# Sudo42b/vision.cpp

Measured on AMD Instinct MI355X. Metric: images/sec, Depth-Anything-V2-Small 518x518 f16, higher is better.
Workload: dtype f16; 1 GPU; Depth-Anything-V2-Small f16 (DINOv2-S ViT) 518x518 batch=32 per MI355X (BASELINE.json configs[1]); global_batch=32, weights=random-init synthetic GGUF (seed 0), parallelism=dp1 (image shards, no data-path collective), hip_graph=True

## Files before the change

### include/visp_hip_kernels.h

```cpp
#ifndef VISP_HIP_KERNELS_H
#define VISP_HIP_KERNELS_H

#include <stddef.h>
#include <stdint.h>

#ifdef __cplusplus
extern "C" {
#endif

#define VX_API __attribute__((visibility("default")))

VX_API const char* vx_last_error(void);
VX_API int vx_device_count(void);
VX_API int vx_set_device(int index);
VX_API int vx_device_info(int index, char* name, int name_cap, char* arch, int arch_cap,
                          size_t* total_mem, size_t* free_mem, int* n_cu);
VX_API int vx_malloc(void** ptr, size_t bytes);
VX_API int vx_free(void* ptr);
VX_API int vx_memset(void* ptr, int value, size_t bytes, void* stream);
VX_API int vx_memcpy_h2d(void* dst, const void* host_src, size_t bytes, void* stream);
VX_API int vx_memcpy_d2h(void* host_dst, const void* src, size_t bytes, void* stream);
VX_API int vx_memcpy_d2d(void* dst, const void* src, size_t bytes, void* stream);
VX_API int vx_malloc_host(void** ptr, size_t bytes);
VX_API int vx_free_host(void* ptr);
VX_API int vx_memcpy_h2d_async(void* dst, const void* pinned_src, size_t bytes, void* stream);
VX_API int vx_memcpy_d2h_async(void* pinned_dst, const void* src, size_t bytes, void* stream);
VX_API int vx_event_sync(void* ev);
VX_API int vx_stream_create(void** stream);
VX_API int vx_stream_destroy(void* stream);
VX_API int vx_stream_sync(void* stream);
VX_API int vx_event_create(void** ev);
VX_API int vx_event_destroy(void* ev);
VX_API int vx_event_record(void* ev, void* stream);
VX_API int vx_event_elapsed_ms(void* start, void* stop, float* ms);
VX_API int vx_stream_wait_event(void* stream, void* ev);
VX_API int vx_graph_begin_capture(void* stream);
VX_API int vx_graph_end_capture(void* stream, void** graph_exec);
VX_API int vx_graph_launch(void* graph_exec, void* stream);
VX_API int vx_graph_destroy(void* graph_exec);

enum vx_epilogue {
    VX_EPI_F16 = 0,
    VX_EPI_F16_GELU = 1,
    VX_EPI_F16_RELU = 2,
    VX_EPI_RESID_F32 = 3,
    VX_EPI_TOKENS = 4,
    VX_EPI_QKV = 5,
    VX_EPI_PIXSHUF = 6,
    VX_EPI_F16_ADD = 7,
    VX_EPI_HEAD_OUT = 8,
    VX_EPI_LRELU_AGC = 9,
    VX_EPI_SILU = 10,
};

typedef struct {
    const void* A;
    int64_t lda;
    int a_group;
    int a_group_stride;
    int a_row_off;
    int conv_kh, conv_kw, conv_stride, conv_pad;
    int conv_H, conv_W, conv_Cin, conv_OH, conv_OW;
    int a_relu;

    const void* W;
    const float* bias;
    int M, N, K;

    int epi;
    void* out;
    int64_t ldo;
    int relu;
    const float* lambda;
    const float* pos;
    int tokens_P;
    void* q; void* k; void* vt;
    int qkv_T, qkv_Tp, qkv_H;
    float q_scale;
    int ps_s, ps_Cout, ps_H, ps_W;
    const void* res1; const void* res2;
    int n_valid;
    int stages;
    float head_bias, head_scale;
    int post_gelu, win_ws, win_res;
    int win_res_h, win_shift;
    int k_splits; float* k_partial;
    void* debug_stamps;
    const float* noise;
    int noise_hw;
    int64_t conv_pix;
    int64_t ld_res1;
} vx_gemm_args;

VX_API int vx_gemm_f16(const vx_gemm_args* args, void* stream);
VX_API int vx_gemm_pick_k_splits(int M, int N, int K);

VX_API int vx_conv3x3_supported(const vx_gemm_args* args);
VX_API int vx_conv3x3_f16(const vx_gemm_args* args, void* stream);

enum { VX_DC_F16 = 0, VX_DC_RGB_F32 = 1, VX_DC_HEAD_F32 = 2 };
typedef struct {
    const void* x; int64_t x_plane; int cin; int up2;
    int B, H, W;
    const void* w; const float* bias; int cout;
    int epi, act;
    float s1; const void* res1; int64_t res1_plane;
    float s2; const void* res2; int64_t res2_plane;
    void* out; int64_t out_plane;
    int x_residual;
    int64_t x_pix, out_pix, res1_pix, res2_pix;
    int a_relu;
    const float* head_w; float head_bias, head_scale;
    void* stamps;
    int bil_hs, bil_ws;
    int res2_hs, res2_ws;
} vx_dconv_args;
VX_API int vx_dconv_bilinear_supported(int cout, int H, int W, int hs, int ws);
VX_API int vx_dconv3x3_f16(const vx_dconv_args* args, void* stream);
VX_API int vx_dconv_prepare(void);
VX_API int vx_dconv_x_residual_supported(float s1, int act, int a_relu);
VX_API int vx_dconv_set_block_cap(int n);
VX_API void vx_dconv_set_resident_mode(int mode);

typedef struct {
    const void* x; const void* w1; const float* b1; const void* w2; const float* b2;
    const void* res2; const void* wp; const float* bp;
    void* out;
    int B, H, W;
} vx_rcu_args;
VX_API int vx_rcu_supported(int H, int W);
VX_API int vx_rcu_fused_f16(const vx_rcu_args* args, void* stream);

typedef struct { int image_w, image_h, overlap_x, overlap_y, n_x, n_y, tile_w, tile_h; } vx_tile_layout;
VX_API int vx_esrgan_tiles_in(const uint8_t* img, int B, int w, int h, int format, const vx_tile_layout* t, void* out, void* stream);
VX_API int vx_esrgan_tiles_in_f32(const uint8_t* img, int B, int w, int h, int format, const vx_tile_layout* t, float* out, void* stream);
VX_API int vx_esrgan_tiles_out(const float* tiles, int B, const vx_tile_layout* t, float* out_f32, uint8_t* out_rgba, void* stream);

VX_API int vx_tv_preprocess(const uint8_t* rgb, void* out, int64_t n_pixels, void* stream);
VX_API int vx_dwconv3x3_f16(const void* x, const void* w, const float* bias, void* y, int B, int H, int W, int C, int stride, int gelu, void* stream);
VX_API int vx_mbconv_dw_pw_supported(int C, int Cout, int W);
VX_API int vx_mbconv_pack_w3(const void* w3_rows_host, void* packed_host);
VX_API int vx_mbconv_dw_pw_f16(const void* h, const void* w2, const float* b2, const void* w3, const float* b3, const void* x, void* y, int B, int H,
                               int W, int C, int Cout, void* stream);
VX_API int vx_layernorm_f16(const void* x, const float* w, const float* b, void* y, int64_t rows_out, int C, float eps, int res, int ws,
                            int out_f32, void* stream);
VX_API size_t vx_window_attention_bias_bytes(int N, int heads);
VX_API int vx_window_attention_pack_bias(const float* bias_host, int N, int heads, void* packed_host);
VX_API int vx_window_attention_f16(const void* qkv, const void* bias_packed, void* out, int n_windows, int N, int heads, void* stream);
VX_API int vx_swin_attention_pack_bias(const float* table , int ws, int heads, void* packed_host );
VX_API int vx_window_attention_masked_f16(const void* qkv, const void* bias_packed, void* out, int n_windows, int N, int heads, int nwx, int nwy,
                                          void* stream);
VX_API int vx_swin_layernorm_f16(const void* x, const float* w, const float* b, void* y, int64_t rows_out, int C, float eps, int H, int W, int ws,
                                 int shift, int out_f32, void* stream);
VX_API int vx_swin_layernorm_strided_f16(const void* x, const float* w, const float* b, void* y, int64_t rows, int C, float eps, int ldy, int out_f32,
                                         void* stream);
VX_API int vx_swin_merge_layernorm_f16(const void* x, const float* w, const float* b, void* y, int B, int H, int W, int C, float eps, void* stream);
VX_API int vx_swin_window_reverse_add_f16(const void* a, const void* x, void* y, int B, int H, int W, int C, int ws, int shift, void* stream);
VX_API int vx_window_reverse_add_f16(const void* a, const void* x, void* y, int B, int res, int ws, int C, void* stream);
VX_API int vx_bf_preprocess_half(const uint8_t* rgb, void* out8, int B, int H, int W, void* stream);
VX_API int vx_bf_patches(const uint8_t* rgb, void* out, int B, int IH, int IW, int h, int w, void* stream);
VX_API int vx_bf_resize_f16(const void* src, int lds, void* dst, int ldd, int B, int h, int w, int C, int oh, int ow, void* stream);
VX_API int vx_bf_deform_cols_f16(const void* x, const void* offmod, int ldom, void* cols, int B, int h, int w, int C, int k, void* stream);
typedef struct {
    const void* x; int B, H, W, Cin;
    const void* w; int Cout, k, pad;
    const void* offset; int ld_offset;
    const void* mask; int ld_mask; int mask_mode; float mask_scale;
    const float* scale; const float* bias; int relu;
    void* out; int ldo;
} vx_deform_conv_args;
VX_API int vx_deform_conv_f16(const vx_deform_conv_args* args, void* stream);
VX_API int vx_bf_mean_f16(const void* x, int ld, void* y, float* acc_scratch , int B, int64_t n, int C, void* stream);
VX_API int vx_bf_broadcast_f16(const void* g, int ldg, void* dst, int ldd, int B, int64_t n, int C, void* stream);
VX_API int vx_bf_mul_sigmoid_f16(void* y, int ldy, const void* a, int lda, int64_t rows, int C, void* stream);
VX_API int vx_bf_sigmoid_out_f32(const void* a, int lda, float* out, int64_t n, void* stream);
VX_API int vx_add_rows_f16(const void* a, int a_is_f32, const void* b, int64_t b_period, void* y, int64_t n, void* stream);
VX_API int vx_small_attention_f16(const void* q, const void* k, const void* v, void* out, int Nq, int Nk, int heads, int hd, void* stream);
VX_API int vx_sam_interpolate(const void* src, int src_f16, int sw, int sh, int sstride, int step, void* dst, int dw, int dh, int out_u8, void* stream);
VX_API int vx_add_gelu_f16(const void* a, const void* b, void* y, int64_t n, void* stream);

#define VX_ATTN_Q_SCALE 0.18033688011112042f
VX_API int vx_attention_f16(const void* q, const void* k, const void* v, void* out, int B, int H, int T,
                            void* stream);
VX_API int vx_attention_masked_f16(const void* q, const void* k, const void* v, const void* mask, void* out, int B, int H, int T, int head_dim,
                                   int Hm, int Bm, int mask_is_f32, void* stream);
VX_API int vx_attention_cross_parts(int Tq, int Tk);
VX_API size_t vx_attention_cross_partial_bytes(int B, int H, int Tq, int Tk, int head_dim);
VX_API int vx_attention_cross_f16(const void* q, const void* k, const void* v, void* out, void* partial, size_t partial_bytes, int B, int H, int Tq, int Tk,
                                  int head_dim, float scale, void* stream);
VX_API int vx_attention_cross_step_f16(int step, const void* q, const void* k, const void* v, void* out, void* partial, size_t partial_bytes, int B, int H, int Tq,
                                       int Tk, int head_dim, float scale, void* stream);
VX_API int vx_mul_mat_f16(const void* a, const void* b, void* out, int64_t M, int N, int K, int B, int Ba, void* stream);
VX_API int vx_sincos_f16(int mode, const void* x, void* y, int64_t n, void* stream);
VX_API int vx_fourier_features_f32(const float* coords, const float* gauss, void* out, int64_t n_points, int F, void* stream);
VX_API int vx_sam_iou_head_f32(const void* tokens, int64_t row_stride, int P, const float* w0, const float* b0, const float* w1, const float* b1, const float* w2,
                               const float* b2, int K0, int N0, int N1, int N2, float* iou, int32_t* chosen, void* stream);
VX_API int vx_sam_process_masks(const void* planes, int64_t prompt_stride, int64_t plane_stride, int step, int mask_size, int n_planes, const int32_t* chosen,
                                float* scaled, int image_size, int sw, int sh, uint8_t* out, int dw, int dh, int P, void* stream);
VX_API int vx_sam_tile_rows_f16(const void* src, int64_t n, void* dst, int B, void* stream);
VX_API int vx_sam_score_planes_f16(const void* planes, int64_t prompt_stride, int64_t plane_stride, int mask_size, int n_planes, int cw, int ch, float offset,
                                   int32_t* table, float* stability, int P, void* stream);
VX_API size_t vx_sam_rank_nms_workspace_bytes(int N);
VX_API int vx_sam_rank_nms(const int32_t* table, const float* iou, int n_planes, int iou_stride, int N, float pred_iou_thresh, float stability_thresh,
                           float nms_iou_thresh, int capacity, void* workspace, size_t workspace_bytes, int32_t* flags, int32_t* rank, int32_t* keep_idx,
                           int32_t* counts, void* stream);
VX_API int vx_sam_process_masks_indexed(const void* planes, int64_t prompt_stride, int64_t plane_stride, int step, int mask_size, int n_scored, int n_prompts,
                                        const int32_t* keep_idx, const int32_t* counts, int capacity, int group, float* scaled, int image_size, int sw, int sh,
                                        uint8_t* out, int dw, int dh, void* stream);
VX_API int vx_sam_mask_stats_u8(const uint8_t* masks, int w, int h, const int32_t* keep_idx, const int32_t* counts, int capacity, int n_scored, int n_prompts,
                                const float* iou, int iou_stride, const float* stability, int32_t* info_i32, float* info_f32, void* stream);
#define VX_REGIONS_HOLES 1
#define VX_REGIONS_ISLANDS 2
#define VX_REGIONS_BOTH 3
VX_API size_t vx_mask_regions_workspace_bytes(int w, int h, int group);
VX_API int vx_mask_remove_small_regions_u8(uint8_t* masks, int w, int h, int n, const int32_t* counts, int min_area, int mode, int32_t* changed, void* workspace,
                                           size_t workspace_bytes, int group, void* stream);
VX_API int vx_sam_clean_nms_inputs(const int32_t* info_i32, const int32_t* changed, const int32_t* counts, int N, int32_t* table, float* key, void* stream);
VX_API int vx_sam_gather_clean_masks(const uint8_t* masks, int w, int h, const int32_t* info_i32, const float* info_f32, const int32_t* changed, const int32_t* keep_idx,
                                     const int32_t* first_counts, const int32_t* second_counts, int N, uint8_t* out_masks, int32_t* out_info_i32, float* out_info_f32,
                                     int32_t* out_counts, void* stream);
VX_API void vx_attention_set_fast_limit(float limit);
VX_API void vx_attention_set_waves(int waves);
VX_API void vx_attention_set_stamps(void* stamps);

typedef struct {
    const void* att; float* x;
    const void* w_mlp; const float* vec_mlp;
    const void* w_qkv; const float* vec_qkv;
    const float* vec_tap; void* feat;
    void *q, *k, *v;
    int M, T, H;
    float q_scale, eps;
    float* cap_x1;
    void* stamps;
} vx_dino_block_args;
VX_API int vx_dino_block_supported(int embed_dim, int hidden, int head_dim);
VX_API size_t vx_dino_block_mlp_bytes(void);
VX_API size_t vx_dino_block_qkv_bytes(void);
VX_API int vx_dino_block16_pack_mlp(const void* wo, const void* w1, const void* w2, void* out);
VX_API int vx_dino_block16_pack_qkv(const void* wqkv, void* out);
VX_API int vx_dino_block16_f16(const vx_dino_block_args* args, void* stream);

typedef struct {
    const void* A; const float* a_scale;
    const void* W; const float* w_scale;
    const float* bias;
    int M, N, Kp, n_valid;
    void* out; int64_t ldo;
    int act;
    const void* res;
} vx_gemm_fp8_args;
VX_API int vx_gemm_fp8_supported(int N, int K);
VX_API int vx_gemm_fp8(const vx_gemm_fp8_args* args, void* stream);
VX_API int vx_quantize_rows_e4m3(const void* x_f16, int64_t ldx, void* q, float* scale, int M, int K, int Kp, void* stream);
VX_API int vx_quantize_rows_e4m3_host(const float* w, int N, int K, int Kp, void* q_out, float* scale_out);

VX_API int vx_layernorm_f32_f16(const float* x, const float* w, const float* b, void* y, int M, int C,
                                float eps, void* stream);

VX_API int vx_preprocess_patches(const uint8_t* rgb, void* patches, int B, int H, int W, int ps, int Kp,
                                 const float mean[3], const float inv_std[3], void* stream);
VX_API int vx_preprocess_f32(const uint8_t* rgb, float* out, int B, int H, int W, const float mean[3],
                             const float inv_std[3], void* stream);
VX_API int vx_write_cls_rows(float* x, const float* cls, const float* pos, int B, int T, int C, void* stream);

VX_API int vx_bilinear_ac_f16(const void* x, void* y, int B, int H, int W, int C, int OH, int OW, void* stream);

VX_API int vx_head_out_f32(const void* x, const float* w, float bias, float max_depth, float* depth,
                           int64_t n_pixels, int C, void* stream);

VX_API size_t vx_headconv_frag_bytes(void);
VX_API int vx_headconv_set_block_cap(int n);
VX_API int vx_headconv_pack(const void* w_rows, int Kp, void* out_frag);
VX_API int vx_headconv_supported(int cin, int cout, int H, int W, int hs, int ws);
VX_API void vx_headconv_set_stamps(void* stamps);
// ... 85 lines not shown
```

### vision.cpp_amd/csrc/kernels_dconv.hip

```cpp
#include "vx_common.h"

#include <cmath>
#include <cstdlib>
#include <type_traits>

namespace {

constexpr int TRASH_BLOCKS = 1024;
__device__ __attribute__((aligned(16))) unsigned char g_dconv_trash[TRASH_BLOCKS * 8 * 1024];

constexpr int DCONV_TAB_MAX = 1280;
constexpr int CK = 32;
constexpr int PIXB = CK * 2;
constexpr int NW = 8;

struct tile_grid {
    int ncols, nrows, n_main, n_strip, strip_x0;
    __host__ __device__ tile_grid(int H, int W) {
        const int q = W / 32, rem = W % 32;
        const bool strip = rem > 0 && rem <= 16;
        ncols = q + ((rem > 16) ? 1 : 0);
        nrows = (H + 15) / 16;
        n_main = ncols * nrows;
        n_strip = strip ? (H + 31) / 32 : 0;
// ... 556 lines not shown
#pragma unroll
                for (int mi = 0; mi < MT; ++mi) {
                    const int oy = cur.y0 + out_row(cur.tws, mi), ox = cur.x0 + out_col(cur.tws);
                    if (oy < H && ox < W) {
                        float* o = reinterpret_cast<float*>(p.out) + (((long)cur.b * H + oy) * W + ox) * 3;
                        o[0] = acc[mi][0][0];
                        o[1] = acc[mi][0][1];
                        o[2] = acc[mi][0][2];
                    }
                }
            }
            wait_vmcnt<0>();
            prev_halo = false;
        } else {
            asm volatile("" ::: "memory");
            __builtin_amdgcn_s_barrier();
            asm volatile("" ::: "memory");
            unsigned char* st;
            if constexpr (COUT == 32) st = smem + done * HALO_BYTES + wave * 64 * PITCH;
            else st = (wave < 4 ? smem + done * HALO_BYTES : smem + W_BASE + WSt * W_BYTES) + (wave & 3) * 64 * PITCH;
            auto stage_tile = [&](auto act_c) {
                constexpr int ACT = decltype(act_c)::value;
#pragma unroll
                for (int mi = 0; mi < MT; ++mi) {
                    const int ml = mi * 32 + r;
#pragma unroll
                    for (int ni = 0; ni < NI; ++ni)
#pragma unroll
                        for (int g = 0; g < 4; ++g) {
                            const int nl = ni * 32 + 8 * g + 4 * h;
                            float4 bias = {0.f, 0.f, 0.f, 0.f};
                            if constexpr (COUT != 32) bias = *reinterpret_cast<const float4*>(s_bias + nl);
                            float v[4] = {acc[mi][ni][4 * g + 0] + bias.x, acc[mi][ni][4 * g + 1] + bias.y,
                                          acc[mi][ni][4 * g + 2] + bias.z, acc[mi][ni][4 * g + 3] + bias.w};
#pragma unroll
                            for (int j = 0; j < 4; ++j) {
                                if constexpr (ACT == 2) v[j] = relu1(v[j]);
                                else if constexpr (ACT == 1) v[j] = fmaxf(v[j], 0.2f * v[j]);
                            }
                            if (xres) {
#pragma unroll
                                for (int j = 0; j < 4; ++j) v[j] *= p.s1;
                            }
                            f16x4 o = {(f16)v[0], (f16)v[1], (f16)v[2], (f16)v[3]};
                            const int c8 = nl >> 2;
                            const int phys16 = (c8 >> 1) ^ stage_swz(ml);
                            *reinterpret_cast<f16x4*>(st + ml * PITCH + phys16 * 16 + (c8 & 1) * 8) = o;
                        }
                }
            };
            if (p.act == 2) stage_tile(std::integral_constant<int, 2>{});
            else if (p.act == 1) stage_tile(std::integral_constant<int, 1>{});
            else stage_tile(std::integral_constant<int, 0>{});
            const char* const R1 = reinterpret_cast<const char*>(p.res1);
            const char* const R2 = reinterpret_cast<const char*>(p.res2);
            constexpr int ROWS_PER_IT = 64 / NCH16, IT_PER_MT = 32 / ROWS_PER_IT;
            constexpr int NB = 4;
            const int j = lane % NCH16, fr0 = lane / NCH16;
            const int jp = j >> 2, je = (j & 3) * 8;
            const bool wide = cur.tws == 5;
            const int oy_b = cur.y0 + (wide ? 2 * wave : 4 * wave), ox_b = cur.x0 + (wide ? fr0 : (fr0 & 15));
            const int tile0 = (cur.b * H + cur.y0) * W + cur.x0;
            const int base = (cur.b * H + oy_b) * W + ox_b;
            const long off1 = ((long)jp * p.res1_plane + je) * 2, off2 = ((long)jp * p.res2_plane + je) * 2, offo = ((long)jp * p.out_plane + je) * 2;
            const bool unit = p.s1 == 1.0f && p.s2 == 1.0f;
            const int rp1 = (int)res1_pix * 2, rp2 = (int)res2_pix * 2, rpo = (int)out_pix * 2;
            wait_lgkmcnt0();
            const float s1 = p.s1, s2 = p.s2;
#pragma unroll
            for (int ib = 0; ib < NCH16; ib += NB) {
                int pixel[NB];
                bool ok[NB];
                f16x8 ra[NB], rc[NB], v[NB];
#pragma unroll
                for (int it = 0; it < NB; ++it) {
                    const int t = ib + it, fm = t / IT_PER_MT, dfr = ROWS_PER_IT * (t % IT_PER_MT);
                    const int dy = wide ? fm : fm + 2 * (dfr >> 4), dx = wide ? dfr : (dfr & 15);
                    ok[it] = oy_b + dy < H && ox_b + dx < W;
                    pixel[it] = ok[it] ? base + dy * W + dx : tile0;
                }
                if (R1) {
#pragma unroll
                    for (int it = 0; it < NB; ++it) ra[it] = *reinterpret_cast<const f16x8*>(R1 + off1 + (long)pixel[it] * rp1);
                }
                if (R2) {
#pragma unroll
                    for (int it = 0; it < NB; ++it) rc[it] = *reinterpret_cast<const f16x8*>(R2 + off2 + (long)pixel[it] * rp2);
                }
#pragma unroll
                for (int it = 0; it < NB; ++it) {
                    const int ml = (ib + it) * ROWS_PER_IT + fr0;
                    v[it] = *reinterpret_cast<const f16x8*>(st + ml * PITCH + (j ^ stage_swz(ml)) * 16);
                }
#pragma unroll
                for (int it = 0; it < NB; ++it) {
                    if (unit) {
                        if (R1) v[it] = v[it] + ra[it];
                        if (R2) v[it] = v[it] + rc[it];
                    } else {
                        if (R1) {
#pragma unroll
                            for (int q = 0; q < 8; ++q) v[it][q] = (f16)((float)v[it][q] * s1 + (float)ra[it][q]);
                        }
                        if (R2) {
#pragma unroll
                            for (int q = 0; q < 8; ++q) v[it][q] = (f16)((float)v[it][q] * s2 + (float)rc[it][q]);
                        }
                    }
                    f16* dst = ok[it] ? reinterpret_cast<f16*>(reinterpret_cast<char*>(p.out) + offo + (long)pixel[it] * rpo) : trash;
                    *reinterpret_cast<f16x8*>(dst) = v[it];
                }
            }
            stores_in_flight = true;
        }
        stamp(4);

        t_cur += t_step;
        if (t_cur >= t_end) return true;
        cur = locate(t_cur);
        if (cur.tws != shape) {
            shape = cur.tws;
            setup_addr(shape);
        }
        zero_acc();
        c = 0;
        stamp(5);
        return false;
    };
    using std::integral_constant;
    for (;;) {
        if constexpr (HS == 3) {
            if (step(integral_constant<int, 0>{}, integral_constant<int, 0>{})) break;
            if (step(integral_constant<int, 1>{}, integral_constant<int, 1>{})) break;
            if (step(integral_constant<int, 2>{}, integral_constant<int, 0>{})) break;
            if constexpr (RES) continue;
            if (step(integral_constant<int, 0>{}, integral_constant<int, 1>{})) break;
            if (step(integral_constant<int, 1>{}, integral_constant<int, 0>{})) break;
            if (step(integral_constant<int, 2>{}, integral_constant<int, 1>{})) break;
        } else {
            if (step(integral_constant<int, 0>{}, integral_constant<int, 0>{})) break;
            if (step(integral_constant<int, 1>{}, integral_constant<int, 1>{})) break;
        }
    }
    if constexpr (STAMP) {
        if (tid == 0) {
            unsigned long long* o = reinterpret_cast<unsigned long long*>(p.stamps) + (size_t)blockIdx.x * 8;
#pragma unroll
            for (int k = 0; k < 6; ++k) o[k] = ph[k];
            o[6] = n_steps;
            o[7] = __builtin_amdgcn_s_memtime();
        }
    }
}

int g_block_cap = 0;
int g_res_mode = -1;

int dconv_grid_blocks() {
    static int n_cu = 0;
    if (g_block_cap > 0) return g_block_cap;
    if (!n_cu) {
        int dev = 0;
        if (hipGetDevice(&dev) != hipSuccess || hipDeviceGetAttribute(&n_cu, hipDeviceAttributeMultiprocessorCount, dev) != hipSuccess || n_cu <= 0) n_cu = 256;
    }
    return n_cu;
}

template <int COUT, int RES, int HSV, bool BIL = false>
constexpr int dconv_smem_bytes() {
    return HSV * (5 * NW * 1024) + (BIL ? 2 * 256 * PIXB : 0) + (RES ? RES : 2) * 9 * COUT * PIXB + (BIL ? ((COUT * 4 + 15) & ~15) + (DCONV_TAB_MAX + 4) * 8 : COUT * 4);
}

template <int COUT, int EPI, bool AR, bool STAMP, int RES = 0, int HSV = (COUT == 32 ? 3 : 2), bool BIL = false, bool ONE = false>
int prepare_variant() {
    static_assert(dconv_smem_bytes<COUT, RES, HSV, BIL>() <= 160 * 1024, "variant does not fit the LDS");
    VX_CHECK(vx_ensure_dynamic_lds(reinterpret_cast<const void*>(&dconv3x3_kernel<COUT, EPI, AR, STAMP, RES, HSV, BIL, ONE>),
                                   dconv_smem_bytes<COUT, RES, HSV, BIL>()));
    return 1;
}

template <int COUT, int EPI, bool AR, bool STAMP, int RES = 0, int HSV = (COUT == 32 ? 3 : 2), bool BIL = false, bool ONE = false>
int launch_variant(const vx_dconv_args& a, hipStream_t s) {
    constexpr int smem = dconv_smem_bytes<COUT, RES, HSV, BIL>();
    if (!prepare_variant<COUT, EPI, AR, STAMP, RES, HSV, BIL, ONE>()) return 0;
    const long tiles = (long)a.B * tile_grid(a.H, a.W).total();
    int blocks = (int)(tiles < dconv_grid_blocks() ? tiles : dconv_grid_blocks());
    if (tiles > dconv_grid_blocks() && dconv_grid_blocks() % 8 == 0) {
        const long per_xcd = (tiles + 7) / 8, cu_per_xcd = dconv_grid_blocks() / 8;
        const long rounds = (per_xcd + cu_per_xcd - 1) / cu_per_xcd;
        const long blocks_per_xcd = (per_xcd + rounds - 1) / rounds;
        blocks = (int)(8 * blocks_per_xcd);
    }
    hipLaunchKernelGGL((dconv3x3_kernel<COUT, EPI, AR, STAMP, RES, HSV, BIL, ONE>), dim3(blocks), dim3(512), smem, s, a);
    VX_LAUNCH_CHECK();
    return 1;
}

template <int COUT, int EPI>
int launch_dconv(const vx_dconv_args& a, hipStream_t s) {
    if constexpr (COUT == 32 && EPI == VX_DC_HEAD_F32) {
        if (a.cin == 32) return a.bil_hs > 0 ? launch_variant<32, EPI, false, false, 0, 2, true, true>(a, s) : launch_variant<32, EPI, false, false, 0, 3, false, true>(a, s);
    }
    if constexpr (COUT == 32 && (EPI == VX_DC_F16 || EPI == VX_DC_HEAD_F32)) {
        if (a.bil_hs > 0) return launch_variant<32, EPI, false, false, 0, 2, true>(a, s);
    }
    if constexpr (EPI == VX_DC_F16) {
        if (a.a_relu) return launch_variant<COUT, EPI, true, false>(a, s);
        if (a.stamps) return launch_variant<COUT, EPI, false, true>(a, s);
        if constexpr (COUT == 32) {
            static const int env_mode = getenv("VISP_DCONV_RES") ? atoi(getenv("VISP_DCONV_RES")) : -1;
            const int res_mode = g_res_mode >= 0 ? g_res_mode : env_mode;
            if (res_mode >= 1 && a.cin == 64) return launch_variant<32, EPI, false, false, 2, 3>(a, s);
            if ((res_mode >= 2 && a.cin <= 128) || (res_mode < 0 && a.cin == 128)) return launch_variant<32, EPI, false, false, 4, 2>(a, s);
        }
    }
    return launch_variant<COUT, EPI, false, false>(a, s);
}


__global__ void esr_tiles_in_kernel(const uint8_t* __restrict__ img, int B, int w, int h, int ch, int ir, int ig, int ib,
                                    vx_tile_layout t, f16* __restrict__ out) {
    const long n = (long)B * t.n_x * t.n_y * t.tile_h * t.tile_w;
    const long i = (long)blockIdx.x * blockDim.x + threadIdx.x;
    if (i >= n) return;
    const int x = (int)(i % t.tile_w);
    long q = i / t.tile_w;
    const int y = (int)(q % t.tile_h);
    q /= t.tile_h;
    const int tile = (int)(q % (t.n_x * t.n_y)), b = (int)(q / (t.n_x * t.n_y));
    const int cx = tile % t.n_x, cy = tile / t.n_x;
    const int sx = min(cx * (t.tile_w - t.overlap_x) + x, w - 1), sy = min(cy * (t.tile_h - t.overlap_y) + y, h - 1);
    const uint8_t* s = img + (((long)b * h + sy) * w + sx) * ch;
    const float v[3] = {(float)s[ir] / 255.0f, (float)s[ig] / 255.0f, (float)s[ib] / 255.0f};
    f16x8* o = reinterpret_cast<f16x8*>(out + i * 32);
    const f16x8 z = {0, 0, 0, 0, 0, 0, 0, 0};
    o[0] = residue_pixel(v);
    o[1] = z;
    o[2] = z;
    o[3] = z;
}

__global__ void esr_tiles_in_f32_kernel(const uint8_t* __restrict__ img, int B, int w, int h, int ch, int ir, int ig, int ib, vx_tile_layout t, float* __restrict__ out) {
    const long n = (long)B * t.n_x * t.n_y * t.tile_h * t.tile_w;
    const long i = (long)blockIdx.x * blockDim.x + threadIdx.x;
    if (i >= n) return;
    const int x = (int)(i % t.tile_w);
    long q = i / t.tile_w;
    const int y = (int)(q % t.tile_h);
    q /= t.tile_h;
    const int tile = (int)(q % (t.n_x * t.n_y)), b = (int)(q / (t.n_x * t.n_y));
    const int cx = tile % t.n_x, cy = tile / t.n_x;
    const int sx = min(cx * (t.tile_w - t.overlap_x) + x, w - 1), sy = min(cy * (t.tile_h - t.overlap_y) + y, h - 1);
    const uint8_t* s = img + (((long)b * h + sy) * w + sx) * ch;
    out[i * 3 + 0] = (float)s[ir] / 255.0f;
    out[i * 3 + 1] = (float)s[ig] / 255.0f;
    out[i * 3 + 2] = (float)s[ib] / 255.0f;
}

__device__ __forceinline__ int tl_start(int c, int tile, int overlap, int pad) { return c * (tile - overlap) + (c == 0 ? 0 : pad); }
__device__ __forceinline__ int tl_end(int c, int n, int tile, int overlap, int pad, int image) {
    const int e = c * (tile - overlap) + tile - (c == n - 1 ? 0 : pad);
    return e < image ? e : image;
}

__global__ void esr_tiles_out_kernel(const float* __restrict__ tiles, int B, vx_tile_layout t, float* __restrict__ out_f32,
                                     uint8_t* __restrict__ out_rgba) {
    const long n = (long)B * t.image_h * t.image_w;
    const long i = (long)blockIdx.x * blockDim.x + threadIdx.x;
    if (i >= n) return;
    const int x = (int)(i % t.image_w);
    const int y = (int)((i / t.image_w) % t.image_h);
    const int b = (int)(i / ((long)t.image_w * t.image_h));
    float d[3] = {0.0f, 0.0f, 0.0f};
    {
#pragma clang fp contract(off)
        for (int cy = 0; cy < t.n_y; ++cy) {
            const int by = tl_start(cy, t.tile_h, t.overlap_y, 0), ey = tl_end(cy, t.n_y, t.tile_h, t.overlap_y, 0, t.image_h);
            if (y < by || y >= ey) continue;
            const int pby = tl_start(cy, t.tile_h, t.overlap_y, t.overlap_y), pey = tl_end(cy, t.n_y, t.tile_h, t.overlap_y, t.overlap_y, t.image_h);
            for (int cx = 0; cx < t.n_x; ++cx) {
                const int bx = tl_start(cx, t.tile_w, t.overlap_x, 0), ex = tl_end(cx, t.n_x, t.tile_w, t.overlap_x, 0, t.image_w);
                if (x < bx || x >= ex) continue;
                const int pbx = tl_start(cx, t.tile_w, t.overlap_x, t.overlap_x), pex = tl_end(cx, t.n_x, t.tile_w, t.overlap_x, t.overlap_x, t.image_w);
                float weight = 1.0f;
                int covx = 0, covy = 0;
                if (x < pbx) { weight *= (float)(t.overlap_x - (pbx - x) + 1); covx = t.overlap_x; }
                else if (x >= pex) { weight *= (float)(t.overlap_x - (x - pex)); covx = t.overlap_x; }
                if (y < pby) { weight *= (float)(t.overlap_y - (pby - y) + 1); covy = t.overlap_y; }
                else if (y >= pey) { weight *= (float)(t.overlap_y - (y - pey)); covy = t.overlap_y; }
                const float* tv = tiles + ((((long)b * t.n_y + cy) * t.n_x + cx) * t.tile_h + (y - by)) * (long)t.tile_w * 3 + (long)(x - bx) * 3;
                if (weight > 0.0f) {
                    const float blend = weight / (float)((covx + 1) * (covy + 1));
                    for (int c = 0; c < 3; ++c) d[c] = d[c] + blend * tv[c];
                } else {
                    for (int c = 0; c < 3; ++c) d[c] = tv[c];
                }
            }
        }
    }
    if (out_f32) {
        out_f32[i * 3 + 0] = d[0];
        out_f32[i * 3 + 1] = d[1];
        out_f32[i * 3 + 2] = d[2];
    }
    if (out_rgba) {
        uchar4 o;
        o.x = (uint8_t)(fminf(fmaxf(d[0], 0.0f), 1.0f) * 255.0f);
        o.y = (uint8_t)(fminf(fmaxf(d[1], 0.0f), 1.0f) * 255.0f);
        o.z = (uint8_t)(fminf(fmaxf(d[2], 0.0f), 1.0f) * 255.0f);
        o.w = 255;
        reinterpret_cast<uchar4*>(out_rgba)[i] = o;
    }
}

}

extern "C" int vx_dconv_prepare(void) {
    return prepare_variant<32, VX_DC_F16, false, false>() && prepare_variant<32, VX_DC_F16, true, false>() &&
           prepare_variant<32, VX_DC_F16, false, false, 2, 3>() && prepare_variant<32, VX_DC_F16, false, false, 4, 2>() &&
           prepare_variant<64, VX_DC_F16, false, false>() && prepare_variant<64, VX_DC_F16, true, false>() &&
           prepare_variant<32, VX_DC_RGB_F32, false, false>() && prepare_variant<32, VX_DC_HEAD_F32, false, false>() &&
           prepare_variant<32, VX_DC_F16, false, false, 0, 2, true>() && prepare_variant<32, VX_DC_HEAD_F32, false, false, 0, 2, true>() &&
           prepare_variant<32, VX_DC_HEAD_F32, false, false, 0, 2, true, true>() && prepare_variant<32, VX_DC_HEAD_F32, false, false, 0, 3, false, true>();
}

extern "C" int vx_dconv_bilinear_supported(int cout, int H, int W, int hs, int ws) {
    if (cout != 32 || H < 2 || W < 2 || hs < 2 || ws < 2 || hs > H || ws > W || H + W > DCONV_TAB_MAX) return 0;
    const double ry = (double)(hs - 1) / (double)(H - 1), rx = (double)(ws - 1) / (double)(W - 1);
    auto rows = [](double r, int n) { return (int)std::floor((n - 1) * r + 1.0) + 2; };
    return rows(ry, 18) <= 12 && rows(rx, 34) <= 21 && rows(ry, 34) <= 21 && rows(rx, 18) <= 12;
}

extern "C" int vx_dconv_set_block_cap(int n) {
    if (n > 0 && (n < 8 || n % 8 != 0)) {
        vx_set_error("vx_dconv_set_block_cap: %d is not a multiple of 8 (one block per XCD at least)", n);
        return 0;
    }
    g_block_cap = n > 0 ? n : 0;
    return 1;
}

extern "C" void vx_dconv_set_resident_mode(int mode) { g_res_mode = mode < 0 ? -1 : mode; }

extern "C" int vx_dconv_x_residual_supported(float s1, int act, int a_relu) {
    if (act != 0 || a_relu || s1 == 0.0f || !std::isfinite(s1)) return 0;
    const float inv = (float)(f16)(1.0f / s1);
    return std::isfinite(inv) && inv * s1 == 1.0f;
}

extern "C" int vx_dconv3x3_f16(const vx_dconv_args* args, void* stream) {
    const vx_dconv_args& a = *args;
    VX_REQUIRE(a.x && a.w && a.out, "vx_dconv3x3_f16: null operand");
    VX_REQUIRE(a.cin >= 32 && a.cin % 32 == 0, "vx_dconv3x3_f16: Cin %d must be a multiple of 32", a.cin);
    VX_REQUIRE(a.B > 0 && a.H > 0 && a.W > 0, "vx_dconv3x3_f16: empty extent");
    VX_REQUIRE((int64_t)a.B * a.H * a.W < (int64_t)0x7fffffff && a.out_pix < (1 << 20) && a.res1_pix < (1 << 20) && a.res2_pix < (1 << 20),
               "vx_dconv3x3_f16: pixel indices must fit 32 bits; run fewer images per call");
    VX_REQUIRE(!a.up2 || (a.H % 2 == 0 && a.W % 2 == 0), "vx_dconv3x3_f16: upsampled extent must be even");
    VX_REQUIRE(a.bil_hs <= 0 || (!a.up2 && !a.a_relu && !a.x_residual && !a.stamps && vx_dconv_bilinear_supported(a.cout, a.H, a.W, a.bil_hs, a.bil_ws)),
               "vx_dconv3x3_f16: bilinear input %dx%d -> %dx%d (cout %d) is outside the interpolating loader's limits", a.bil_ws, a.bil_hs, a.W, a.H, a.cout);
    VX_REQUIRE(a.res2_hs <= 0, "vx_dconv3x3_f16: bilinear res2 is not built");
    VX_REQUIRE((reinterpret_cast<uintptr_t>(a.x) & 15) == 0 && (reinterpret_cast<uintptr_t>(a.w) & 15) == 0 &&
               (reinterpret_cast<uintptr_t>(a.out) & 15) == 0, "vx_dconv3x3_f16: operands must be 16-byte aligned");
    {
        const int64_t src_pixels = a.bil_hs > 0 ? (int64_t)a.bil_hs * a.bil_ws : (int64_t)(a.H >> (a.up2 ? 1 : 0)) * (a.W >> (a.up2 ? 1 : 0));
        const int64_t xp = a.x_pix ? a.x_pix : 32;
        VX_REQUIRE(xp >= 32 && xp % 8 == 0 && a.out_pix % 8 == 0 && a.res1_pix % 8 == 0 && a.res2_pix % 8 == 0, "vx_dconv3x3_f16: pixel strides must be multiples of 8 (input >= 32)");
        VX_REQUIRE(a.cin == 32 || (a.x_plane % 8 == 0 && (xp > 32 ? a.x_plane >= 32 : a.x_plane >= (int64_t)a.B * src_pixels * 32)), "vx_dconv3x3_f16: bad input plane stride");
        VX_REQUIRE((int64_t)(a.cin / 32 - 1) * a.x_plane * 2 + src_pixels * xp * 2 < (int64_t)0x7fffffff,
                   "vx_dconv3x3_f16: input planes span more than 2 GiB; run fewer images per call");
    }
    hipStream_t s = as_stream(stream);
    if (a.epi == VX_DC_RGB_F32) {
        VX_REQUIRE(a.cout == 32 && !a.a_relu, "vx_dconv3x3_f16: the rgb head takes weights padded to 32 outputs");
        VX_REQUIRE(a.act == 0 && !a.res1 && !a.res2 && !a.x_residual, "vx_dconv3x3_f16: the rgb head has no activation and no residuals");
        return launch_dconv<32, VX_DC_RGB_F32>(a, s);
    }
    if (a.epi == VX_DC_HEAD_F32) {
        VX_REQUIRE(a.cout == 32 && a.head_w && !a.a_relu, "vx_dconv3x3_f16: the fused depth head is a 32-channel epilogue with head_w set");
        VX_REQUIRE(a.act == 0 && !a.res1 && !a.res2 && !a.x_residual, "vx_dconv3x3_f16: the fused depth head applies its own ReLUs and takes no residuals");
        return launch_dconv<32, VX_DC_HEAD_F32>(a, s);
    }
    VX_REQUIRE(a.epi == VX_DC_F16, "vx_dconv3x3_f16: unknown epilogue %d", a.epi);
    VX_REQUIRE(a.out_plane % 8 == 0 && a.res1_plane % 8 == 0 && a.res2_plane % 8 == 0, "vx_dconv3x3_f16: plane strides must be multiples of 8");
    VX_REQUIRE(!a.x_residual || (a.cout == 64 && a.cin >= 64 && !a.res1 && !a.up2 && a.s1 != 0.0f),
               "vx_dconv3x3_f16: x_residual needs cout = 64 <= cin, no res1, no upsampling");
    VX_REQUIRE(!a.x_residual || vx_dconv_x_residual_supported(a.s1, a.act, a.a_relu),
               "vx_dconv3x3_f16: x_residual needs act = 0, no a_relu and an s1 = %g whose reciprocal is exact in f16; pass x as res1", (double)a.s1);
    VX_REQUIRE(a.act >= 0 && a.act <= 2, "vx_dconv3x3_f16: unknown activation %d", a.act);
    if (a.cout == 32) return launch_dconv<32, VX_DC_F16>(a, s);
    if (a.cout == 64) return launch_dconv<64, VX_DC_F16>(a, s);
    vx_set_error("vx_dconv3x3_f16: Cout %d not in {32, 64}", a.cout);
    return 0;
}

extern "C" int vx_esrgan_tiles_in(const uint8_t* img, int B, int w, int h, int format, const vx_tile_layout* t, void* out, void* stream) {
    int ch, ir, ig, ib;
    switch (format) {
        case 0: ch = 4; ir = 0; ig = 1; ib = 2; break;
        case 1: ch = 4; ir = 2; ig = 1; ib = 0; break;
        case 2: ch = 4; ir = 1; ig = 2; ib = 3; break;
        case 3: ch = 3; ir = 0; ig = 1; ib = 2; break;
        default: vx_set_error("vx_esrgan_tiles_in: unsupported image format %d", format); return 0;
    }
    const long n = (long)B * t->n_x * t->n_y * t->tile_h * t->tile_w;
    hipLaunchKernelGGL(esr_tiles_in_kernel, dim3((unsigned)((n + 255) / 256)), dim3(256), 0, as_stream(stream), img, B, w, h, ch, ir, ig, ib, *t,
                       reinterpret_cast<f16*>(out));
    VX_LAUNCH_CHECK();
    return 1;
}

extern "C" int vx_esrgan_tiles_in_f32(const uint8_t* img, int B, int w, int h, int format, const vx_tile_layout* t, float* out, void* stream) {
    int ch, ir, ig, ib;
    switch (format) {
        case 0: ch = 4; ir = 0; ig = 1; ib = 2; break;
        case 1: ch = 4; ir = 2; ig = 1; ib = 0; break;
        case 2: ch = 4; ir = 1; ig = 2; ib = 3; break;
        case 3: ch = 3; ir = 0; ig = 1; ib = 2; break;
        default: vx_set_error("vx_esrgan_tiles_in_f32: unsupported image format %d", format); return 0;
    }
    const long n = (long)B * t->n_x * t->n_y * t->tile_h * t->tile_w;
    hipLaunchKernelGGL(esr_tiles_in_f32_kernel, dim3((unsigned)((n + 255) / 256)), dim3(256), 0, as_stream(stream), img, B, w, h, ch, ir, ig, ib, *t, out);
    VX_LAUNCH_CHECK();
    return 1;
}

extern "C" int vx_esrgan_tiles_out(const float* tiles, int B, const vx_tile_layout* t, float* out_f32, uint8_t* out_rgba, void* stream) {
    const long n = (long)B * t->image_h * t->image_w;
    hipLaunchKernelGGL(esr_tiles_out_kernel, dim3((unsigned)((n + 255) / 256)), dim3(256), 0, as_stream(stream), tiles, B, *t, out_f32, out_rgba);
    VX_LAUNCH_CHECK();
    return 1;
}
```

Measured before the change: 6510 images/s.

## Add weight-stationary 64-channel 3x3 conv kernel with per-XCD tile scheduling

Adds a new HIP kernel for 64-in/64-out f16 3x3 convolutions that keeps each wave's 16-output-channel weight slice in registers. It streams 16x32 input halo tiles into LDS via buffer loads and walks the tile rows with MFMA accumulation and a fused bias, activation and residual epilogue. Tiles are split across XCDs so each XCD takes a contiguous range, with up to two blocks per CU. The new path is picked by default only when there is no block cap, no residuals and enough tiles per image, and it is otherwise reachable through an env var or setter. It gives up the existing resident dconv path's weight-in-LDS design for that case, and adds register pressure and extra kernel variants.

```diff
diff --git a/include/visp_hip_kernels.h b/include/visp_hip_kernels.h
--- a/include/visp_hip_kernels.h
+++ b/include/visp_hip_kernels.h
@@ -121,6 +121,10 @@
 VX_API int vx_dconv_x_residual_supported(float s1, int act, int a_relu);
 VX_API int vx_dconv_set_block_cap(int n);
 VX_API void vx_dconv_set_resident_mode(int mode);
+VX_API int vx_dconv_ws_supported(const vx_dconv_args* args);
+VX_API void vx_dconv_set_weight_stationary(int mode);
+VX_API int vx_dconv_ws_selected(const vx_dconv_args* args, int n_cu, int block_cap);
+VX_API void vx_dconv_ws_set_stamps(void* stamps);
 
 typedef struct {
     const void* x; const void* w1; const float* b1; const void* w2; const float* b2;
diff --git a/vision.cpp_amd/csrc/kernels_dconv.hip b/vision.cpp_amd/csrc/kernels_dconv.hip
--- a/vision.cpp_amd/csrc/kernels_dconv.hip
+++ b/vision.cpp_amd/csrc/kernels_dconv.hip
@@ -732,6 +732,13 @@
         }
     }
 }
+
+}
+
+int dconv_ws_prepare();
+int dconv_ws_launch(const vx_dconv_args& a, hipStream_t s, int n_cu);
+
+namespace {
 
 int g_block_cap = 0;
 int g_res_mode = -1;
@@ -901,7 +908,8 @@
            prepare_variant<64, VX_DC_F16, false, false>() && prepare_variant<64, VX_DC_F16, true, false>() &&
            prepare_variant<32, VX_DC_RGB_F32, false, false>() && prepare_variant<32, VX_DC_HEAD_F32, false, false>() &&
            prepare_variant<32, VX_DC_F16, false, false, 0, 2, true>() && prepare_variant<32, VX_DC_HEAD_F32, false, false, 0, 2, true>() &&
-           prepare_variant<32, VX_DC_HEAD_F32, false, false, 0, 2, true, true>() && prepare_variant<32, VX_DC_HEAD_F32, false, false, 0, 3, false, true>();
+           prepare_variant<32, VX_DC_HEAD_F32, false, false, 0, 2, true, true>() && prepare_variant<32, VX_DC_HEAD_F32, false, false, 0, 3, false, true>() &&
+           dconv_ws_prepare();
 }
 
 extern "C" int vx_dconv_bilinear_supported(int cout, int H, int W, int hs, int ws) {
@@ -968,7 +976,10 @@
                "vx_dconv3x3_f16: x_residual needs act = 0, no a_relu and an s1 = %g whose reciprocal is exact in f16; pass x as res1", (double)a.s1);
     VX_REQUIRE(a.act >= 0 && a.act <= 2, "vx_dconv3x3_f16: unknown activation %d", a.act);
     if (a.cout == 32) return launch_dconv<32, VX_DC_F16>(a, s);
-    if (a.cout == 64) return launch_dconv<64, VX_DC_F16>(a, s);
+    if (a.cout == 64) {
+        if (vx_dconv_ws_selected(&a, dconv_grid_blocks(), g_block_cap)) return dconv_ws_launch(a, s, dconv_grid_blocks());
+        return launch_dconv<64, VX_DC_F16>(a, s);
+    }
     vx_set_error("vx_dconv3x3_f16: Cout %d not in {32, 64}", a.cout);
     return 0;
 }
diff --git a/vision.cpp_amd/csrc/kernels_dconv_ws.hip b/vision.cpp_amd/csrc/kernels_dconv_ws.hip
--- /dev/null
+++ b/vision.cpp_amd/csrc/kernels_dconv_ws.hip
@@ -0,0 +1,275 @@
+#include <algorithm>
+#include <cstdlib>
+#include <utility>
+
+#include "vx_common.h"
+
+namespace {
+
+constexpr int TH = 16, TW = 32, HH = TH + 2, HW = TW + 2;
+constexpr int HALO_PIX = HH * HW;
+constexpr int N_BLK16 = (HALO_PIX + 15) / 16;
+constexpr int HALO_BYTES = N_BLK16 * 2048;
+constexpr int N_PIECES = HALO_BYTES / 1024;
+constexpr int PJ = (N_PIECES + 3) / 4;
+constexpr int SMEM_BYTES = HALO_BYTES;
+static_assert(2 * SMEM_BYTES <= 160 * 1024, "two blocks per CU");
+
+template <class F, int... I>
+__device__ __forceinline__ void static_for_impl(F&& f, std::integer_sequence<int, I...>) { (f(std::integral_constant<int, I>{}), ...); }
+template <int N, class F>
+__device__ __forceinline__ void static_for(F&& f) { static_for_impl(f, std::make_integer_sequence<int, N>{}); }
+
+typedef short s16x8 __attribute__((ext_vector_type(8)));
+__device__ __forceinline__ f16x8 relu_f16x8(f16x8 v) {
+    return __builtin_bit_cast(f16x8, __builtin_elementwise_max(__builtin_bit_cast(s16x8, v), s16x8{0, 0, 0, 0, 0, 0, 0, 0}));
+}
+
+constexpr int RD = 4;
+template <bool AR, int NRES, bool STAMP>
+__global__ __launch_bounds__(256) __attribute__((amdgpu_waves_per_eu(2, 2))) void dconv_ws_kernel(const vx_dconv_args p, int tiles_x, int tiles_y,
+                                                                                                   unsigned long long* __restrict__ stamps) {
+    extern __shared__ __attribute__((aligned(16))) unsigned char smem[];
+    const int tid = threadIdx.x, lane = tid & 63;
+    const int wave = __builtin_amdgcn_readfirstlane(tid >> 6);
+    const int px = lane & 15, q = lane >> 4;
+    const int H = p.H, W = p.W;
+    const int per_image = tiles_x * tiles_y, total = p.B * per_image;
+
+    int t_cur, t_end, t_step;
+    {
+        const int id = blockIdx.x, xcd = id & 7;
+        const int per = total >> 3, rem = total & 7;
+        const int lo = xcd < rem ? xcd * (per + 1) : rem * (per + 1) + (xcd - rem) * per;
+        t_end = lo + per + (xcd < rem ? 1 : 0);
+        t_step = ((int)gridDim.x - xcd + 7) >> 3;
+        t_cur = lo + (id >> 3);
+    }
+    if (t_cur >= t_end) return;
+
+    f16x8 wf[18];
+    {
+        const f16* const w = reinterpret_cast<const f16*>(p.w);
+        const int n = 16 * wave + px;
+#pragma unroll
+        for (int tap = 0; tap < 9; ++tap)
+#pragma unroll
+            for (int kb = 0; kb < 2; ++kb) wf[tap * 2 + kb] = *reinterpret_cast<const f16x8*>(w + ((size_t)(kb * 9 + tap) * 64 + n) * 32 + ((q ^ ((n >> 2) & 3)) * 8));
+    }
+    const int ch0 = 16 * wave + 4 * q;
+    f32x4 bias4 = {0.f, 0.f, 0.f, 0.f};
+    if (p.bias) bias4 = *reinterpret_cast<const f32x4*>(p.bias + ch0);
+
+    const int x_pix = (int)p.x_pix;
+    const long img_bytes = (long)H * W * x_pix * 2;
+    const int act_floor = p.act == 2 ? 0 : (int)0x80000000;
+    const int rp1 = (int)p.res1_pix * 2, rp2 = (int)p.res2_pix * 2, rpo = (int)p.out_pix * 2;
+
+    unsigned bt[16];
+#pragma unroll
+    for (int r = 0; r < 16; ++r) bt[r] = (unsigned)(((r + px) >> 4) * 2048 + ((r + px) & 15) * 16 + q * 256);
+
+    typedef unsigned u32x2 __attribute__((ext_vector_type(2)));
+    const int npix = p.B * H * W;
+    const __amdgpu_buffer_rsrc_t o_rsrc = __builtin_amdgcn_make_buffer_rsrc(p.out, 0, (npix - 1) * rpo + 128, 0x00020000);
+    const __amdgpu_buffer_rsrc_t r1_rsrc = __builtin_amdgcn_make_buffer_rsrc(const_cast<void*>(p.res1), 0, NRES > 0 ? (npix - 1) * rp1 + 128 : 0, 0x00020000);
+    const __amdgpu_buffer_rsrc_t r2_rsrc = __builtin_amdgcn_make_buffer_rsrc(const_cast<void*>(p.res2), 0, NRES > 1 ? (npix - 1) * rp2 + 128 : 0, 0x00020000);
+    constexpr unsigned OOB = 0x80000000u;
+
+    unsigned long long st[2] = {0, 0}, c0 = 0;
+    const unsigned long long t_start = STAMP ? __builtin_amdgcn_s_memtime() : 0;
+    int n_done = 0;
+
+    for (; t_cur < t_end; t_cur += t_step, ++n_done) {
+        const int b = t_cur / per_image, k = t_cur - b * per_image, ty = k / tiles_x;
+        const int y0 = ty * TH, x0 = (k - ty * tiles_x) * TW;
+        if constexpr (STAMP) c0 = __builtin_amdgcn_s_memtime();
+
+        {
+            const __amdgpu_buffer_rsrc_t x_rsrc =
+                __builtin_amdgcn_make_buffer_rsrc(const_cast<char*>(reinterpret_cast<const char*>(p.x)) + b * img_bytes, 0, (int)img_bytes, 0x00020000);
+            int l = lane;
+            asm volatile("" : "+v"(l));
+#pragma unroll
+            for (int j = 0; j < PJ; ++j) {
+                const int piece = wave + 4 * j;
+                if (piece < N_PIECES) {
+                    const int s = piece * 64 + l;
+                    const int pix = (s >> 7) * 16 + (s & 15), c = (s >> 4) & 7;
+                    const int hy = pix / HW, hx = pix - hy * HW;
+                    const int iy = y0 - 1 + hy, ix = x0 - 1 + hx;
+                    const bool valid = pix < HALO_PIX && (unsigned)iy < (unsigned)H && (unsigned)ix < (unsigned)W;
+                    const unsigned off = valid ? (unsigned)(((iy * W + ix) * x_pix + c * 8) * 2) : 0x80000000u;
+                    __builtin_amdgcn_raw_ptr_buffer_load_lds(x_rsrc, (lptr_t)(smem + piece * 1024), 16, off, 0, 0, 0);
+                }
+            }
+        }
+        wait_vmcnt<0>();
+        __syncthreads();
+        if constexpr (STAMP) {
+            const unsigned long long c = __builtin_amdgcn_s_memtime();
+            st[0] += c - c0;
+            c0 = c;
+        }
+
+        f32x4 acc[3][2];
+        f16x8 bf[2][6];
+        unsigned vo[2], v1[2], v2[2];
+#pragma unroll
+        for (int g = 0; g < 2; ++g) {
+            const bool okc = x0 + g * 16 + px < W;
+            vo[g] = okc ? (unsigned)((g * 16 + px) * rpo + ch0 * 2) : OOB;
+            v1[g] = okc ? (unsigned)((g * 16 + px) * rp1 + ch0 * 2) : OOB;
+            v2[g] = okc ? (unsigned)((g * 16 + px) * rp2 + ch0 * 2) : OOB;
+        }
+        const int pix0 = (b * H + y0) * W + x0;
+        f16x4 rv[RD + 1][2];
+        auto load_group = [&](int s, f16x8 (&r)[6]) {
+            const int hr = s >> 1, g = s & 1;
+#pragma unroll
+            for (int kx = 0; kx < 3; ++kx) {
+                const int first = hr * HW + g * 16 + kx;
+                const unsigned a = bt[first & 15] + (unsigned)((first >> 4) * 2048);
+#pragma unroll
+                for (int kb = 0; kb < 2; ++kb) {
+                    r[kx * 2 + kb] = *reinterpret_cast<const f16x8*>(smem + a + kb * 1024);
+                }
+            }
+        };
+        load_group(0, bf[0]);
+        static_for<2 * HH>([&](auto s_c) __attribute__((always_inline)) {
+            constexpr int s = decltype(s_c)::value;
+            constexpr int hr = s >> 1, g = s & 1, j_out = hr - 2, j_slot = (j_out + 3) % 3;
+            if (s + 1 < 2 * HH) load_group(s + 1, bf[(s + 1) & 1]);
+            if constexpr (NRES > 0 && s + RD < 2 * HH && (s + RD) / 2 >= 2) {
+                constexpr int gn = (s + RD) & 1, jn = (s + RD) / 2 - 2;
+                const bool row_ok = y0 + jn < H;
+                const int pn = pix0 + jn * W;
+                rv[(s + RD) % (RD + 1)][0] = __builtin_bit_cast(f16x4, __builtin_amdgcn_raw_buffer_load_b64(r1_rsrc, row_ok ? v1[gn] : OOB, pn * rp1, 0));
+                if constexpr (NRES > 1)
+                    rv[(s + RD) % (RD + 1)][1] = __builtin_bit_cast(f16x4, __builtin_amdgcn_raw_buffer_load_b64(r2_rsrc, row_ok ? v2[gn] : OOB, pn * rp2, 0));
+            }
+            __builtin_amdgcn_sched_barrier(0);
+            if constexpr (AR) {
+#pragma unroll
+                for (int f = 0; f < 6; ++f) bf[s & 1][f] = relu_f16x8(bf[s & 1][f]);
+            }
+#pragma unroll
+            for (int kx = 0; kx < 3; ++kx)
+#pragma unroll
+                for (int kb = 0; kb < 2; ++kb)
+#pragma unroll
+                    for (int dy = 0; dy < 3; ++dy) {
+                        const int j = hr - dy;
+                        if (j >= 0 && j < TH) {
+                            const bool first = dy == 0 && kx == 0 && kb == 0;
+                            const f32x4 c = first ? f32x4{0.f, 0.f, 0.f, 0.f} : acc[j % 3][g];
+                            acc[j % 3][g] = __builtin_amdgcn_mfma_f32_16x16x32_f16(wf[(dy * 3 + kx) * 2 + kb], bf[s & 1][kx * 2 + kb], c, 0, 0, 0);
+                        }
+                    }
+            if constexpr (j_out >= 0) {
+                const f32x4 a4 = acc[j_slot][g];
+                float v[4] = {a4[0] + bias4[0], a4[1] + bias4[1], a4[2] + bias4[2], a4[3] + bias4[3]};
+#pragma unroll
+                for (int e = 0; e < 4; ++e) v[e] = __int_as_float(max(__float_as_int(v[e]), act_floor));
+                f16x4 o = {(f16)v[0], (f16)v[1], (f16)v[2], (f16)v[3]};
+                if constexpr (NRES > 0) o = o + rv[s % (RD + 1)][0];
+                if constexpr (NRES > 1) o = o + rv[s % (RD + 1)][1];
+                __builtin_amdgcn_raw_buffer_store_b64(__builtin_bit_cast(u32x2, o), o_rsrc, y0 + j_out < H ? vo[g] : OOB, (pix0 + j_out * W) * rpo, 0);
+            }
+            __builtin_amdgcn_sched_barrier(0);
+        });
+        if constexpr (STAMP) st[1] += __builtin_amdgcn_s_memtime() - c0;
+        __syncthreads();
+    }
+    if constexpr (STAMP) {
+        if (lane == 0) {
+            unsigned long long* o = stamps + ((size_t)blockIdx.x * 4 + wave) * 4;
+            o[0] = st[0]; o[1] = st[1]; o[2] = (unsigned long long)n_done; o[3] = __builtin_amdgcn_s_memtime() - t_start;
+        }
+    }
+}
+
+int g_ws_mode = -1;
+int ws_mode() {
+    static const int env_mode = getenv("VISP_DCONV_WS") ? (atoi(getenv("VISP_DCONV_WS")) ? 1 : 0) : -1;
+    return g_ws_mode >= 0 ? g_ws_mode : env_mode;
+}
+void* g_ws_stamps = nullptr;
+
+template <bool AR, int NRES, bool STAMP>
+int launch_ws(const vx_dconv_args& a, hipStream_t s, int blocks, int tiles_x, int tiles_y) {
+    VX_CHECK(vx_ensure_dynamic_lds(reinterpret_cast<const void*>(&dconv_ws_kernel<AR, NRES, STAMP>), SMEM_BYTES));
+    hipLaunchKernelGGL((dconv_ws_kernel<AR, NRES, STAMP>), dim3(blocks), dim3(256), SMEM_BYTES, s, a, tiles_x, tiles_y, static_cast<unsigned long long*>(g_ws_stamps));
+    VX_LAUNCH_CHECK();
+    return 1;
+}
+
+long ws_tiles(const vx_dconv_args& a) { return (long)a.B * ((a.W + TW - 1) / TW) * ((a.H + TH - 1) / TH); }
+
+}
+
+int dconv_ws_prepare() {
+    const void* const kernels[] = {reinterpret_cast<const void*>(&dconv_ws_kernel<false, 0, false>), reinterpret_cast<const void*>(&dconv_ws_kernel<false, 1, false>),
+                                   reinterpret_cast<const void*>(&dconv_ws_kernel<false, 2, false>), reinterpret_cast<const void*>(&dconv_ws_kernel<true, 0, false>),
+                                   reinterpret_cast<const void*>(&dconv_ws_kernel<true, 1, false>), reinterpret_cast<const void*>(&dconv_ws_kernel<true, 2, false>)};
+    for (const void* k : kernels) VX_CHECK(vx_ensure_dynamic_lds(k, SMEM_BYTES));
+    return 1;
+}
+
+int dconv_ws_blocks(long tiles, int n_cu) {
+    const long most = 2L * n_cu;
+    if (tiles <= most || most % 8 != 0) return (int)std::min(tiles, most);
+    const long per_xcd = (tiles + 7) / 8, slots = most / 8;
+    const long rounds = (per_xcd + slots - 1) / slots;
+    return (int)(8 * ((per_xcd + rounds - 1) / rounds));
+}
+
+namespace {
+template <bool AR, bool STAMP>
+int launch_ws_res(const vx_dconv_args& a, hipStream_t s, int blocks, int tiles_x, int tiles_y) {
+    if (a.res1 && a.res2) return launch_ws<AR, 2, STAMP>(a, s, blocks, tiles_x, tiles_y);
+    if (!a.res1 && !a.res2) return launch_ws<AR, 0, STAMP>(a, s, blocks, tiles_x, tiles_y);
+    vx_dconv_args one = a;
+    if (!one.res1) {
+        one.res1 = a.res2; one.res1_pix = a.res2_pix; one.res1_plane = a.res2_plane;
+        one.res2 = nullptr;
+    }
+    return launch_ws<AR, 1, STAMP>(one, s, blocks, tiles_x, tiles_y);
+}
+}
+
+int dconv_ws_launch(const vx_dconv_args& a, hipStream_t s, int n_cu) {
+    const int tiles_x = (a.W + TW - 1) / TW, tiles_y = (a.H + TH - 1) / TH;
+    const int blocks = dconv_ws_blocks(ws_tiles(a), n_cu);
+    if (g_ws_stamps) return a.a_relu ? launch_ws_res<true, true>(a, s, blocks, tiles_x, tiles_y) : launch_ws_res<false, true>(a, s, blocks, tiles_x, tiles_y);
+    return a.a_relu ? launch_ws_res<true, false>(a, s, blocks, tiles_x, tiles_y) : launch_ws_res<false, false>(a, s, blocks, tiles_x, tiles_y);
+}
+
+extern "C" int vx_dconv_ws_supported(const vx_dconv_args* args) {
+    const vx_dconv_args& a = *args;
+    if (a.epi != VX_DC_F16 || a.cin != 64 || a.cout != 64) return 0;
+    if (a.x_plane != 32 || a.x_pix < 64 || a.out_plane != 32 || a.out_pix < 64) return 0;
+    if (a.res1 && (a.res1_plane != 32 || a.res1_pix < 64)) return 0;
+    if (a.res2 && (a.res2_plane != 32 || a.res2_pix < 64)) return 0;
+    if (a.x_pix % 8 || a.out_pix % 8 || (a.res1 && a.res1_pix % 8) || (a.res2 && a.res2_pix % 8)) return 0;
+    if (a.up2 || a.bil_hs > 0 || a.res2_hs > 0 || a.x_residual || a.stamps) return 0;
+    if (a.s1 != 1.0f || a.s2 != 1.0f || (a.act != 0 && a.act != 2)) return 0;
+    if (a.B <= 0 || a.H <= 0 || a.W <= 0 || (int64_t)a.H * a.W * a.x_pix * 2 >= (int64_t)0x7fffffff) return 0;
+    const int64_t npix = (int64_t)a.B * a.H * a.W;
+    if (npix * a.out_pix * 2 >= (int64_t)0x7fffffff || (a.res1 && npix * a.res1_pix * 2 >= (int64_t)0x7fffffff) ||
+        (a.res2 && npix * a.res2_pix * 2 >= (int64_t)0x7fffffff)) return 0;
+    return 1;
+}
+
+extern "C" void vx_dconv_set_weight_stationary(int mode) { g_ws_mode = mode < 0 ? -1 : (mode ? 1 : 0); }
+
+extern "C" int vx_dconv_ws_selected(const vx_dconv_args* args, int n_cu, int block_cap) {
+    const int mode = ws_mode();
+    if (mode == 0 || !vx_dconv_ws_supported(args)) return 0;
+    if (mode == 1) return 1;
+    (void)n_cu;
+    return block_cap <= 0 && !args->res1 && !args->res2 && ws_tiles(*args) / args->B >= 32;
+}
+
+extern "C" void vx_dconv_ws_set_stamps(void* stamps) { g_ws_stamps = stamps; }
```

New measurement: 6563 images/s, median of 6. No clear change (+0.8%).
